# lesterphillip/SVCC23_FastSVC

Measured on AMD Instinct MI355X. Metric: audio samples/sec (24 kHz) FastSVC generator fwd, higher is better.
Workload: dtype bf16 (bf16 MFMA products, f32 accumulate; bf16 storage); 1 GPU; cfg3: 64 x 10 s utterances per GPU, F=1500 frames, T=240000 samples, generator fastsvc.yaml (144->[192,96,48,24], x[2,4,4,5]), spk_emb on; global_batch=64, utterance_samples=240000, parallelism=utterance-parallel x1

## Files before the change

### include/fastsvc_hip.h

```cpp
#ifndef FASTSVC_HIP_H
#define FASTSVC_HIP_H

#include <stddef.h>
#include <stdint.h>

#ifdef __cplusplus
extern "C" {
#endif

#define FASTSVC_ABI_VERSION 1
#define FASTSVC_MAX_STAGES 8

enum {
    FASTSVC_OK = 0,
    FASTSVC_E_INVALID = -1,
    FASTSVC_E_MISSING = -2,
    FASTSVC_E_WORKSPACE = -3,
    FASTSVC_E_HIP = -4,
    FASTSVC_E_UNSUPPORTED = -5
};

typedef struct fastsvc_config {
    int32_t in_channels;
    int32_t n_stages;
    int32_t mid_channels[FASTSVC_MAX_STAGES];
    int32_t upsampling_scales[FASTSVC_MAX_STAGES];
    int32_t out_channels;
    int32_t spk_emb_size;
    int32_t use_spk_emb;
} fastsvc_config;

typedef struct fastsvc_tensor {
    const char* name;
    const float* data;
    int64_t numel;
} fastsvc_tensor;

typedef struct fastsvc_plan fastsvc_plan;

int fastsvc_abi_version(void);
const char* fastsvc_last_error(void);

int fastsvc_plan_create(const fastsvc_config* cfg, fastsvc_plan** out_plan);
void fastsvc_plan_destroy(fastsvc_plan* plan);

int fastsvc_plan_set_storage(fastsvc_plan* plan, int32_t dtype);
int fastsvc_plan_get_storage(const fastsvc_plan* plan);

size_t fastsvc_weight_blob_bytes(const fastsvc_plan* plan);

int fastsvc_pack_weights(const fastsvc_plan* plan, const fastsvc_tensor* tensors, int32_t n_tensors,
                         void* host_blob);

size_t fastsvc_pack_device_scratch_bytes(const fastsvc_plan* plan);
int fastsvc_pack_device_launch_count(const fastsvc_plan* plan);
int fastsvc_pack_weights_device(const fastsvc_plan* plan, const fastsvc_tensor* tensors, int32_t n_tensors,
                                void* dev_blob, void* scratch, size_t scratch_bytes, void* stream);

int fastsvc_plan_set_workspace_mode(fastsvc_plan* plan, int32_t compact);

size_t fastsvc_workspace_bytes(const fastsvc_plan* plan, int32_t B, int32_t F);

int fastsvc_forward(const fastsvc_plan* plan, const void* dev_blob,
                    const float* ppg, const float* sine, const float* lft, const float* spk_emb,
                    float* out, int32_t B, int32_t F, const int32_t* lengths,
                    void* workspace, size_t workspace_bytes, void* stream);

int fastsvc_stream_prepare(void* stream);

int fastsvc_stream_release(void* stream);
// ... 122 lines not shown
```

### svcc23_fastsvc_amd/csrc/fastsvc_hx.hip

```cpp
#include "fastsvc_kernels.h"

namespace fastsvc {
#ifdef FASTSVC_ACT_2B
namespace FASTSVC_ACT_NS {
#endif

#include "fastsvc_device.inc"

#include "fastsvc_hx_common.inc"

template <int MW, int NW, bool RELOAD, bool OPT_LAST = false, int NS = 3 * MW * HX_NP, int SOFF = 0, bool ADV = true, bool HOLD = false>
__device__ __forceinline__ void hx_unit_direct(f32x4 (&acc)[NW][MW], const unsigned char* tile, const int (&aoff)[3],
                                               int lo_off, HxWeightStream<NS>& ws, bool do_last = true, bool hold = false) {
    constexpr int NSTEP = 3 * NW;
    constexpr int PF = HX_NP == 1 ? (MW >= 3 ? 2 : 3) : 1;
    HxFrag a[PF + 1];
    #pragma unroll
    for (int q = 0; q < PF && q < NSTEP; ++q) a[q] = hx_read(tile, aoff[q / NW] + (q % NW) * 16 * HX_ROW, lo_off);
    #pragma unroll
    for (int s = 0; s < NSTEP; ++s) {
        const int tap = s / NW, n = s % NW;
        if (s + PF < NSTEP) {
            a[(s + PF) % (PF + 1)] = hx_read(tile, aoff[(s + PF) / NW] + ((s + PF) % NW) * 16 * HX_ROW, lo_off);
            __builtin_amdgcn_sched_barrier(0);
// ... 436 lines not shown
            v += __builtin_bit_cast(float, __builtin_amdgcn_mov_dpp(__builtin_bit_cast(int, v), 0x4E, 0xF, 0xF, true));
            v += __builtin_bit_cast(float, __builtin_amdgcn_mov_dpp(__builtin_bit_cast(int, v), 0x141, 0xF, 0xF, true));
            v += __builtin_bit_cast(float, __builtin_amdgcn_mov_dpp(__builtin_bit_cast(int, v), 0x140, 0xF, 0xF, true));
            s[e] = v;
        }
        const int t = PAIRS ? tcol0 + (n >> 1) * 32 + (lane >> 4) * 8 + (n & 1) * 4 : tcol0 + n * 16 + (lane >> 4) * 4;
        buf_store4(yr, ((lane & 15) == 0 && t < p.T) ? t * 4 : OOB_OFF, s + bias);
    }
}

#ifndef FASTSVC_HX_W8
#define FASTSVC_HX_W8 1
#endif
constexpr bool hx_w8(int MODE, bool tailk, int S) {
    return FASTSVC_HX_W8 != 0 && HX_NP == 1 && !tailk && (MODE == MODE_DIRECT || MODE == MODE_POLY || (MODE == MODE_DEC2 && S == 2));
}
#ifndef FASTSVC_HX_CARRY
#define FASTSVC_HX_CARRY 1
#endif
constexpr bool hx_carry(int MODE, bool tailk, int S, int NT) {
    return FASTSVC_HX_CARRY != 0 && hx_w8(MODE, tailk, S) && MODE == MODE_DIRECT && S == 1 && NT == 128;
}

template <int MW, int NW, int WM, int WN, int MODE, int EPI, int S, bool WSTATIC, bool TAILK = false>
__global__ __launch_bounds__(512, (hx_min_waves<MW, NW, MODE, EPI, S, TAILK>()))
void conv_hx_kernel(const ConvParams p0) {
    constexpr bool UPH = MODE == MODE_UPHEAD;
    constexpr bool POLY = MODE == MODE_POLY, DEC2 = MODE == MODE_DEC2, CHAIN = MODE == MODE_CHAIN || MODE == MODE_CHAIN1 || UPH;
    constexpr bool IN1 = MODE == MODE_CHAIN1;
    constexpr bool WLB = MODE == MODE_CHAIN && S == 2;
    constexpr bool XR = MODE == MODE_DIRECT && S > 1;
    constexpr int NT = 16 * NW * WN;
    constexpr int NTV = CHAIN ? NT + 16 : NT;
    constexpr int HB = CHAIN ? 4 : 0;
    constexpr int NPROD_T = 256;
    constexpr bool W8 = hx_w8(MODE, TAILK, S);
    constexpr int SPARE = W8 ? 8 : 4;
    constexpr int MAXW = NTV + (MODE == MODE_DIRECT ? (W8 ? 64 : 56) : (W8 ? 16 : 8));
    constexpr int ITEMS = (MAXW + NPROD_T - 1) / NPROD_T;
    constexpr int NWS = DEC2 ? 4 : 3;
    constexpr int NVAR = DEC2 ? 2 : 1;
    constexpr int NSLOT = NWS * MW * HX_NP;
    constexpr bool TRACKS = AMAX_TRACK && ((CHAIN && MODE != MODE_UPHEAD) || (MODE == MODE_DIRECT && (EPI == EPI_RES || EPI == EPI_RANK1)));
    extern __shared__ __attribute__((aligned(16))) unsigned char smem_raw[];

    const int tid = threadIdx.x;
// ... 5 lines not shown
    const int wave_n = cw - wave_m * WN;
    const int z = blockIdx.z;
    const int sig = z / p0.B;
    const int b = z - sig * p0.B;
    ConvParams p = p0;
    if (p0.lens) {
        const int frames = p0.lens[b];
        p.T = frames * p0.len_mul;
        p.x_T = frames * p0.xlen_mul;
    }
    const int mg = blockIdx.y * WM + wave_m;
    const bool active = !producer && mg < p.ngroups;
    const int halo = (MODE == MODE_DIRECT || CHAIN) ? p.dil : 1;
    const int halo_al = W8 ? ((halo + 7) & ~7) : ((halo + 3) & ~3);
    const int W = NTV + 2 * halo_al;
    const int nch = p.nch32;
    const int CINp = nch * HX_KC;
    const int flags = p.flags;
    const int ntx = (p.T + NT - 1) / NT;
    const int tile0 = blockIdx.x * p.tpw;
    const int ntiles = min(p.tpw, ntx - tile0);
    if (ntiles <= 0) return;
    const int nunits = ntiles * (XR ? 2 * nch : nch);
#ifdef FASTSVC_TIMELINE
    const int wg_lin = blockIdx.x + gridDim.x * (blockIdx.y + gridDim.y * blockIdx.z);
    unsigned long long* tlw = (p.tl && wg_lin < p.tl_wgs) ? p.tl + ((long)wg_lin * 8 + wave) * 64 : nullptr;
    int tli = 0;
    auto stamp = [&](int tag) {
        if (tlw && lane == 0 && tli < 62) { tlw[tli++] = ((unsigned long long)tag << 56) | (__builtin_readcyclecounter() & 0x00ffffffffffffffull); }
    };
    stamp(1);
    if (tlw && lane == 0) {
        tlw[62] = __builtin_amdgcn_s_getreg(4 | (0 << 6) | (31 << 11));
        tlw[63] = __builtin_amdgcn_s_getreg(20 | (0 << 6) | (31 << 11));
    }
#else
    auto stamp = [](int) {};
#endif

    if constexpr (hx_min_waves<MW, NW, MODE, EPI, S, TAILK>() >= 4) {
        const int wg_id = blockIdx.x + gridDim.x * (blockIdx.y + gridDim.y * blockIdx.z);
        if ((wg_id >> 8) & 1) {
            for (int k = 0; k < p.stagger; ++k) __builtin_amdgcn_s_sleep(16);
        }
    }
    double* sstat = reinterpret_cast<double*>(smem_raw);
// ... 465 lines not shown
                    #pragma unroll
                    for (int m = 0; m < MW; ++m) { s1p[m] = 0.f; s2p[m] = 0.f; }
                    if (pact) P2.request(p, Rp, mg, tcolw, lane);
                    __syncthreads();
                    if (pact) {
                        P2.run(p, Rp, Pw, s1p, s2p, mg, tcolw, lane);
                        if (flags & F_STATS) {
                            #pragma unroll
                            for (int m = hx_poly_mc<MW>(); m < MW; ++m) {
                                if (lane < 16) {
                                    const int slot = ((wave_m * MW + m) * 16 + lane) * 2;
                                    atomicAdd(&sstat[slot + 0], (double)s1p[m]);
                                    atomicAdd(&sstat[slot + 1], (double)s2p[m]);
                                }
                            }
                        }
                    }
                }
            }
#endif
        };
        pwin_t pa[ITEMS][8], pb[ITEMS][8];
        unsigned oka = 0, okb = 0;
        bool carried = false;
#ifdef FASTSVC_ACT_2B
        if constexpr (hx_carry(MODE, TAILK, S, NT)) {
            carried = p.tpw > 1 && nch <= 2 && 2 * halo_al <= NT && 8 * halo_al <= NPROD_T;
            if (carried) {
                const int f_pair = ptid & 15, f_oct = ptid >> 4;
                const int f_row = 2 * halo_al + 8 * f_oct;
                auto ploadF = [&](int un, act4_t (&px)[4], unsigned& nv) {
                    const int tl = l_tl, ch = l_ch;
                    pos_next(l_tl, l_ch);
                    const int t = (tile0 + tl) * NT - halo_al + f_row;
                    const int soff = ch * HX_KC * p.ldx * 4;
                    const int rows_left = p.CIN - ch * HX_KC;
                    const bool live = ((unsigned)t < (unsigned)p.T) & (un < nunits) & !(FASTSVC_DBG_ON(p, DBG_NO_LOAD));
                    nv = live ? (unsigned)min(8, p.T - t) : 0u;
                    #pragma unroll
                    for (int c = 0; c < 2; ++c) {
                        const int r = f_pair * 2 + c;
                        typedef unsigned u32x4w __attribute__((ext_vector_type(4)));
                        const u32x4w w = __builtin_amdgcn_raw_buffer_load_b128(xr, (live & (r < rows_left)) ? (r * p.ldx + t) * 2 : OOB_OFF, soff >> 1, FASTSVC_LD_AUX);
                        px[2 * c] = act4_t{w.x, w.y};
                        px[2 * c + 1] = act4_t{w.z, w.w};
                    }
                };
                auto pcommitF = [&](const act4_t (&pw)[4], unsigned nvi, unsigned char* tile) {
                    if (FASTSVC_DBG_ON(p, DBG_NO_COMMIT)) return;
                    const int ch = c_ch;
// ... 11 lines not shown
                    }
                    #pragma unroll
                    for (int j = 0; j < 8; ++j) {
                        float e[2];
                        #pragma unroll
                        for (int c = 0; c < 2; ++c) e[c] = px[2 * c + (j >> 2)][j & 3] * A[c] + Bc[c];
                        if (j >= 4 && row_end) {
                            #pragma unroll
                            for (int c = 0; c < 2; ++c) e[c] = nvi > 4 ? e[c] : 0.f;
                        }
                        #pragma unroll
                        for (int c = 0; c < 2; ++c) e[c] = fmaxf(e[c], e[c] * slope);
                        *reinterpret_cast<unsigned*>(tile + hx_lds_off(f_row + j, f_pair >> 2) + (f_pair & 3) * 4) = a16_pack2(e[0], e[1]);
                        __builtin_amdgcn_sched_barrier(0);
                    }
                };
                const bool c_live = ptid < 8 * halo_al;
                const int c_src = NT * HX_ROW + (c_live ? ptid : 0) * 16;
                const int c_dst = c_live ? ptid * 16 : W * HX_ROW + (ptid & 31) * 16;
                auto cread = [&](const unsigned char* buf) -> u32x4 { return *reinterpret_cast<const u32x4*>(buf + c_src); };
                auto cwrite = [&](unsigned char* buf, const u32x4& v) { *reinterpret_cast<u32x4*>(buf + c_dst) = v; };
                act4_t fa[4], fb[4];
                unsigned na = 0, nb = 0;
                if (nch == 1) {
                    pload(0, pa, oka);
                    ploadF(1, fb, nb);
                    stamp(2);
                    setup_shared();
                    pcommit(0, pa, oka, tiles);
                    stamp(3);
                    __syncthreads();
                    stamp(4);
                    for (int u = 0; u < nunits; u += 2) {
                        const u32x4 ca = cread(tiles);
                        ploadF(u + 2, fa, na);
                        stamp(9);
                        cwrite(tiles + bufsz, ca);
                        pcommitF(fb, nb, tiles + bufsz);
                        stamp(5);
                        __syncthreads();
                        stamp(6);
                        const u32x4 cb = cread(tiles + bufsz);
                        ploadF(u + 3, fb, nb);
                        stamp(9);
                        cwrite(tiles, cb);
                        pcommitF(fa, na, tiles);
                        stamp(5);
// ... 26 lines not shown
                    stamp(6);
                    for (int u = 2; u < nunits; u += 2) {
                        ca = cread(tiles);
                        ploadF(u + 2, fa, na);
                        stamp(9);
                        cwrite(tiles + bufsz, cb);
                        pcommitF(fb, nb, tiles + bufsz);
                        stamp(5);
                        __syncthreads();
                        stamp(6);
                        cb = cread(tiles + bufsz);
                        ploadF(u + 3, fb, nb);
                        stamp(9);
                        cwrite(tiles, ca);
                        pcommitF(fa, na, tiles);
                        stamp(5);
                        __syncthreads();
                        stamp(6);
                    }
                }
            }
        }
#endif
        if (!carried) {
        pload(0, pa, oka);
        pload(1, pb, okb);
        stamp(2);
        setup_shared();
        if constexpr (IN1 && HX_NP == 2) {
            #pragma unroll
            for (int c = 0; c < 8; ++c) { i1w[c][0] *= sx; i1w[c][1] *= sx; i1w[c][2] *= sx; i1b[c] *= sx; }
        }
        pcommit(0, pa, oka, tiles);
        stamp(3);
        __syncthreads();
        stamp(4);
        for (int u = 0; u < nunits; u += 2) {
            pload(u + 2, pa, oka);
            stamp(9);
            pcommit(u + 1, pb, okb, tiles + bufsz);
            stamp(5);
            ppass2(u);
            __syncthreads();
            if (CHAIN && (u % nch) == nch - 1) __syncthreads();
            stamp(6);
            pload(u + 3, pb, okb);
            stamp(9);
// ... 447 lines not shown
                }
                stamp(8);
                __syncthreads();
                stamp(6);
            }
        }
        if constexpr (TRACKS) amax_flush(p, R, &s_amax, &s_cnt, 4, sig, b, lane, blockIdx.x);
        if constexpr (GSTAT || TWO) {
            if ((flags & F_STATS) && !(FASTSVC_DBG_ON(p, DBG_NO_EPILOGUE))) {
                #pragma unroll
                for (int m = 0; m < MW; ++m) {
                    double a1 = g1[GSTAT ? m : 0], a2 = g2[GSTAT ? m : 0];
                    if constexpr (TWO) { a1 = Gw[(2 * m) * 64]; a2 = Gw[(2 * m + 1) * 64]; }
                    a1 += __shfl_xor(a1, 16); a2 += __shfl_xor(a2, 16);
                    a1 += __shfl_xor(a1, 32); a2 += __shfl_xor(a2, 32);
                    if (active && lane < 16) {
                        const int slot = ((wave_m * MW + m) * 16 + lane) * 2;
                        atomicAdd(&sstat[slot + 0], a1);
                        atomicAdd(&sstat[slot + 1], a2);
                    }
                }
            }
        }
        if (nunits & 1) __syncthreads();
    }
    if ((flags & F_STATS) && !(FASTSVC_DBG_ON(p, DBG_NO_EPILOGUE))) {
        __syncthreads();
        for (int i = tid; i < 2 * 16 * MW * WM; i += 512) {
            const int co = blockIdx.y * (WM * MW * 16) + (i >> 1);
            if (co < p.COUT) atomicAdd(&p.st_out[((long)b * p.COUT + co) * 2 + (i & 1)], sstat[i]);
        }
    }
}

constexpr size_t HX_STATIC_LDS = 4096;
template <auto KERNEL>
static hipError_t hx_launch_instance(dim3 grid, size_t smem, hipStream_t stream, const ConvParams& p) {
    if (smem + HX_STATIC_LDS > 64 * 1024) {
        static const hipError_t attr = hipFuncSetAttribute(reinterpret_cast<const void*>(KERNEL),
                                                           hipFuncAttributeMaxDynamicSharedMemorySize, 160 * 1024 - HX_STATIC_LDS);
        if (attr != hipSuccess) return attr;
    }
    hipLaunchKernelGGL(KERNEL, grid, dim3(512), smem, stream, p);
    return hipGetLastError();
}

// ... 171 lines not shown
```

### svcc23_fastsvc_amd/csrc/fastsvc_kernels.h

```cpp
#pragma once
#include <hip/hip_runtime.h>
#include <stdint.h>

#if defined(FASTSVC_ACT_BF16) && defined(FASTSVC_ACT_F16)
#error "FASTSVC_ACT_BF16 and FASTSVC_ACT_F16 exclude each other"
#endif
#if defined(FASTSVC_ACT_BF16)
#define FASTSVC_ACT_2B 1
#define FASTSVC_ACT_NS bf16
#elif defined(FASTSVC_ACT_F16)
#define FASTSVC_ACT_2B 1
#define FASTSVC_ACT_NS f16
#endif

namespace fastsvc {

enum : int {
    MODE_DIRECT = 0,
    MODE_DECIMATE = 1,
    MODE_STRETCH = 2,
    MODE_POLY = 3,
    MODE_WINO = 4,
    MODE_DEC2 = 5,
    MODE_CHAIN = 6,
// ... 62 lines not shown
    long bias2_sig;
    const float* res;
    long res_sig, res_b;
    const float* r1x;
    long r1x_sig, r1x_b;
    const float* r1w;
    const float* r1b;
    long r1_sig;
    const float* ss_in;
    long ss_in_b;
    const double* st_in;
    const float* spk;
    const float* ss_out;
    long ss_out_b;
    double* st_out;
    int ntaps, dil, mode, s, flags;
    int B;
    int xs;
    int ps;
    int ldx, ldy;
    const int* lens;
    int len_mul, xlen_mul;
    int frames_ld;
    unsigned long long* tl;
    int tl_wgs;
    int vec;
    int tpw;
    int dbg;
};

struct CondStage0Params {
    const float* x;
    long x_sig, x_b;
    int B, C, T, ld;
    const int* lens;
    int len_mul;
    const float* in1_w[2];
    const float* in1_b[2];
    const float* r1w[2];
    const float* r1b[2];
    const void* w[3][2];
    const float* bias[3][2];
    const float* winv[3][2];
    const float* bnd[4][2];
    const float* bnd_r[2];
    const float* cbnd[2];
// ... 125 lines not shown
```

### svcc23_fastsvc_amd/csrc/fastsvc_plan.cpp

```cpp
#include <hip/hip_runtime.h>

#include <algorithm>
#include <chrono>
#include <cmath>
#include <cstddef>
#include <cstdio>
#include <cstdlib>
#include <cstring>
#include <functional>
#include <map>
#include <mutex>
#include <thread>
#include <type_traits>
#include <atomic>
#include <string>
#include <unordered_map>
#include <vector>

#include "fastsvc_hip.h"
#include "fastsvc_kernels.h"
#include "fastsvc_pack.h"

using namespace fastsvc;

// ... 3 lines not shown

int fail(int code, const std::string& msg) {
    g_err = msg;
    return code;
}

inline size_t align_up(size_t v, size_t a) { return (v + a - 1) / a * a; }

struct Switches {
    static int num(const char* name, int dflt) { const char* v = std::getenv(name); return v ? std::atoi(v) : dflt; }
    static double real(const char* name, double dflt) { const char* v = std::getenv(name); return v ? std::atof(v) : dflt; }
    static bool given(const char* name) { return std::getenv(name) != nullptr; }
    const int hx = num("FASTSVC_HX", 1);
    const int wx = num("FASTSVC_WX", 1);
    const int wino = num("FASTSVC_WINO", -1);
    const int chain = num("FASTSVC_CHAIN", 1);
    const int uphead = num("FASTSVC_UPHEAD", 1);
    const int d3x = num("FASTSVC_D3X", 1);
    const bool no_poly = given("FASTSVC_NO_POLY");
    const bool no_dec2 = given("FASTSVC_NO_DEC2");
    const bool no_fuse_last = given("FASTSVC_NO_FUSE_LAST");
    const int prior = num("FASTSVC_PRIOR", 1);
    const double startup_us = real("FASTSVC_STARTUP_US", 4.0);
    const int stagger = num("FASTSVC_STAGGER", 2);
    const int dbg = num("FASTSVC_DBG", 0);
    const int cond = num("FASTSVC_COND", 1);
    const int cond_pipe = num("FASTSVC_COND_PIPE", 1);
    const int cond_small = num("FASTSVC_COND_SMALL", -1);
    const int cond_tpw = num("FASTSVC_COND_TPW", 0);
    const int cond1_tpw = num("FASTSVC_COND1_TPW", 0);
    const int cond_dbg = num("FASTSVC_COND_DBG", 0);
    const bool cond_trace = given("FASTSVC_COND_TRACE");
    const bool no_amax_scan = given("FASTSVC_NO_AMAX_SCAN");
    const bool serial = given("FASTSVC_SERIAL");
    const int streams = num("FASTSVC_STREAMS", -1);
    const double fork_join_limit_us = real("FASTSVC_FORK_JOIN_LIMIT_US", 40.0);
    const bool stream_debug = given("FASTSVC_STREAM_DEBUG");
    const int pack_threads = num("FASTSVC_PACK_THREADS", 0);
    const bool pack_debug = given("FASTSVC_PACK_DEBUG");
    const bool verbose_shapes = given("FASTSVC_VERBOSE_SHAPES");
};
const Switches& env() {
    static const Switches s;
    return s;
}

// ... 127 lines not shown
}

struct fastsvc_plan {
    fastsvc_config cfg;
    int n = 0;
    std::vector<int> down_scales;
    std::vector<DownStage> down;
    std::vector<UpStage> up;
    RawParam last;
    size_t blob_floats = 0;
    std::vector<std::pair<PackedConv*, PackSource>> pack_jobs;
    struct ChainJob { PackedConv* c; std::string first, second, in1; };
    std::vector<ChainJob> chain_jobs;
    struct FilmChainJob { PackedConv* c; std::string conv[2]; PackSource heads; int C; };
    std::vector<FilmChainJob> film_chain_jobs;
    struct UpHeadJob { PackedConv* c; std::string first, res, up; int cin, C; };
    std::vector<UpHeadJob> up_head_jobs;
    struct XrJob { PackedConv* c; std::string conv, res; };
    std::vector<XrJob> xr_jobs;
    std::vector<RawParam*> raw_jobs;
    std::vector<int> cond_bound_jobs;
    double flops_per_sample = 0.0;
    int storage = 0;
    bool compact = false;
    struct Choice { int NW, WM, WN, tpw, algo; };
    mutable std::mutex tune_mu;
    mutable std::map<std::string, Choice> tuned;
    mutable std::map<std::string, Choice> priors;
    mutable std::vector<double> pack_cost;
    PackTable pk;
    mutable std::once_flag pk_once;
    mutable void* pk_pinned = nullptr;
    ~fastsvc_plan() { if (pk_pinned) (void)hipHostFree(pk_pinned); }

    bool prior_for(const char* layer, int B, int T, bool two_byte, Choice& out) const {
        const size_t ln = std::strlen(layer);
        double best = 1e30;
        bool found = false;
        for (const auto& kv : tuned) {
            const std::string& k = kv.first;
            if (k.size() <= ln + 1 || k.compare(0, ln, layer) != 0 || k[ln] != '|') continue;
            int b = 0, t = 0;
            char tail = 0;
            const int n = std::sscanf(k.c_str() + ln + 1, "%d|%d|%c", &b, &t, &tail);
            if (n < 2 || b <= 0 || t <= 0 || (n == 3) != two_byte) continue;
            const double d = std::fabs(std::log((double)b * t / ((double)B * T))) + 0.25 * std::fabs(std::log((double)t / T));
// ... 1389 lines not shown
    if (hipGetDevice(&dev) != hipSuccess) return 0;
    ExecCtx* c = nullptr;
    {
        std::lock_guard<std::mutex> lock(g_ctx_mu);
        auto it = g_ctxs.find(std::make_pair(dev, stream));
        if (it == g_ctxs.end()) return 0;
        c = it->second;
        g_ctxs.erase(it);
    }
    {
        std::lock_guard<std::mutex> busy(c->busy);
        for (hipStream_t a : c->aux)
            if (a) { (void)hipStreamSynchronize(a); (void)hipStreamDestroy(a); }
        for (hipEvent_t e : c->ev)
            if (e) (void)hipEventDestroy(e);
    }
    delete c;
    return 1;
}

struct CallCtx {
    const fastsvc_plan* plan = nullptr;
    int storage = 0;
    bool tuning = false;
    int trials = 0;
    bool exact_f32 = false;
};

#ifdef FASTSVC_TIMELINE
template <class LaunchFn>
bool timeline_launch(const char* layer, ConvParams& p, long wgs, int nchunks, const ConvLaunch& L, hipStream_t stream,
                     LaunchFn&& fn, hipError_t& err) {
    const char* want = std::getenv("FASTSVC_TIMELINE_LAYER");
    const char* out = std::getenv("FASTSVC_TIMELINE_OUT");
    if (!want || !out || std::strcmp(want, layer) != 0) return false;
    const long cap = wgs < 8192 ? wgs : 8192;
    unsigned long long* dbuf = nullptr;
    const size_t bytes = (size_t)cap * 8 * 64 * sizeof(unsigned long long);
    if (hipMalloc(&dbuf, bytes) != hipSuccess) { err = hipErrorOutOfMemory; return true; }
    hipMemsetAsync(dbuf, 0, bytes, stream);
    p.tl = dbuf; p.tl_wgs = (int)cap;
    err = fn();
    if (err != hipSuccess) return true;
    hipStreamSynchronize(stream);
    std::vector<unsigned long long> host((size_t)cap * 8 * 64);
    hipMemcpy(host.data(), dbuf, bytes, hipMemcpyDeviceToHost);
// ... 893 lines not shown
static int forward_impl(CallCtx& cc, const fastsvc_plan* plan, const void* dev_blob,
                    const float* ppg, const float* sine, const float* lft, const float* spk_emb,
                    float* out, int32_t B, int32_t F, const int32_t* lengths,
                    void* workspace, size_t workspace_bytes, void* stream_, Profiler* prof) {
    if (!plan || !dev_blob || !ppg || !sine || !lft || !out || !workspace)
        return fail(FASTSVC_E_INVALID, "null argument");
    if (B < 1 || F < 1) return fail(FASTSVC_E_INVALID, "B and F must be >= 1");
    const fastsvc_plan& P = *plan;
    if (P.storage != 0) {
        const std::string mode = P.storage == 2 ? "float16 storage" : "bfloat16 storage";
        if (F % 4 != 0) return fail(FASTSVC_E_UNSUPPORTED, mode + " needs a frame count that is a multiple of 4");
        for (int k = 0; k < P.n; ++k)
            if (P.down[k].c2[0].KC != 24 || P.up[k].d3.KC != 24 || P.up[k].first.KC != 24)
                return fail(FASTSVC_E_UNSUPPORTED, mode + " needs the pipelined kernels (24-channel K chunks)");
        if (P.n > 1 && !P.down[1].rc1[0].dec2) return fail(FASTSVC_E_UNSUPPORTED, mode + " needs the fused decimating pair");
    }
    if (spk_emb && !P.cfg.use_spk_emb)
        return fail(FASTSVC_E_INVALID, "spk_emb given but the generator was built with use_spk_emb=False");
    const Workspace ws = layout_workspace(P, B, F);
    if (workspace_bytes < ws.bytes) return fail(FASTSVC_E_WORKSPACE, "workspace too small");
    hipStream_t stream = static_cast<hipStream_t>(stream_);
    cc.plan = plan;
    cc.storage = plan->storage;
    cc.exact_f32 = plan->storage == 0 && F <= 4;
    int64_t hop_all = 1;
    for (int i = 0; i < plan->n; ++i) hop_all *= plan->cfg.upsampling_scales[i];
    int streams_mask = env().serial ? 0 : env().streams >= 0 ? (env().streams & 3) : ((int64_t)B * F * hop_all >= 150000 ? 2 : 0);
    ExecCtx* ctx = (streams_mask == 0 || cc.tuning || prof) ? nullptr : exec_ctx_for(stream);
    std::unique_lock<std::mutex> ctx_lock;
    if (ctx) {
        ctx_lock = std::unique_lock<std::mutex>(ctx->busy);
        ensure_measured(stream, ctx);
        if (env().streams < 0 && !ctx->pays) { ctx_lock.unlock(); ctx_lock = std::unique_lock<std::mutex>(); ctx = nullptr; streams_mask = 0; }
    }
    hipStream_t s_film = (ctx && (streams_mask & 2)) ? ctx->aux[0] : stream;
    hipStream_t s_side = (ctx && (streams_mask & 1)) ? ctx->aux[1] : stream;
    int evi = 0;
    auto order_after = [&](hipStream_t from, hipStream_t to) -> hipError_t {
        if (from == to || !ctx) return hipSuccess;
        hipEvent_t e = ctx->ev[evi++ % ctx->ev.size()];
        hipError_t r = hipEventRecord(e, from);
        if (r != hipSuccess) return r;
        return hipStreamWaitEvent(to, e, 0);
    };
    std::vector<hipEvent_t> ss_ready(P.n, nullptr);
    const float* blob = static_cast<const float*>(dev_blob);
// ... 57 lines not shown
                                      4.0 * (spk_c * P.cfg.spk_emb_size + (double)B * P.cfg.spk_emb_size + spk_c * B)));
        HIP_TRY(launch_spk_proj(spk_emb, blocks, n, B, P.cfg.spk_emb_size, s_pre));
        if (prof) HIP_TRY(prof->end());
    }

    long Tk = T;
    const float* hprev = sigbuf;
    int Cprev = 1;
    long Tprev = T;
    bool hprev_compact = false;
    for (int k = 0; k < n; ++k) {
        const DownStage& d = P.down[k];
        Tk = Tk / d.scale;
        const std::string s = std::to_string(k);
        float* c1 = buf("down_c1." + s);
        float* c2 = buf("down_c2." + s);
        float* h = buf("down_h." + s);
        const long tsig = (long)B * d.C * Tk;
        const long tb = (long)d.C * Tk;
        ConvParams base;
        std::memset(&base, 0, sizeof(base));
        base.B = B; base.T = (int)Tk; base.s = 1; base.mode = MODE_DIRECT;
        base.lens = lengths; base.frames_ld = F;
        base.amax_in_sig = B; base.amax_out_sig = B;
        float* am_prev = k == 0 ? amax_inb : am("down_h." + std::to_string(k - 1));
        float* am_h = am("down_h." + s);
        const float* bnd_c1 = blob + (k == 0 ? d.c1_raw[0].bnd_off : d.c1[0].bnd_off);
        const long bnd_c1_sig = k == 0 ? (long)(d.c1_raw[1].bnd_off - d.c1_raw[0].bnd_off) : d.c1[0].bnd_pair;
        auto stage_unfused = [&](Profiler* pr) -> int {
            if (k == 0) {
                if (pr) HIP_TRY(pr->begin(stream, "down.0.c1", "in1_conv", 2.0 * 3 * d.C * (double)Tk * B * 2,
                                              4.0 * (1.0 + d.C) * (double)Tk * B * 2));
                HIP_TRY(FASTSVC_BY_STORAGE(P.storage, launch_in1_conv)(sigbuf, sig_stride, blob + d.c1_raw[0].w_off, blob + d.c1_raw[0].b_off,
                                        (long)(d.c1_raw[1].w_off - d.c1_raw[0].w_off),
                                        (long)(d.c1_raw[1].b_off - d.c1_raw[0].b_off), c1, 2, B, d.C, (int)Tk,
                                        lengths, (int)(Tk / F), stream, nullptr));
                if (pr) HIP_TRY(pr->end());
            } else {
                float* r = buf("down_r." + s);
                ConvParams p = base;
                p.x = hprev; p.x_sig = (long)B * Cprev * Tprev; p.x_b = (long)Cprev * Tprev; p.x_T = (int)Tprev;
                p.mode = MODE_DECIMATE; p.s = hprev_compact ? 1 : d.scale;
                p.amax_in = am_prev;
                if (d.rc1[0].dec2 && !env().no_dec2) {
                    p.mode = MODE_DEC2;
                    p.y = c1; p.y_sig = tsig; p.y_b = tb;
// ... 149 lines not shown
        if (env().no_fuse_last || (table_entry(P, key, ch) && ch.algo != 3)) last_fusable = false;
    }
    for (int i = 0; i < n; ++i) {
        const UpStage& u = P.up[i];
        const int k = n - 1 - i;
        const long Tout = Tin * u.scale;
        const std::string s = std::to_string(i);
        float* a = buf("up." + s + ".a");
        float* xr = buf("up." + s + ".xr");
        float* u1 = buf("up." + s + ".u1");
        float* xm = buf("up." + s + ".xmid");
        float* u2 = buf("up." + s + ".u2");
        float* u3 = buf("up." + s + ".u3");
        float* xo = buf("up." + s + ".out");
        float* pb = buf("up." + s + ".spk");
        double* st = reinterpret_cast<double*>(buf("up." + s + ".stats"));
        const float* ss = buf("ss." + std::to_string(k));
        const long cb = (long)u.C * Tout;
        const long stn = (long)B * u.C * 2;
        ConvParams base;
        std::memset(&base, 0, sizeof(base));
        base.B = B; base.s = 1; base.mode = MODE_DIRECT;
        base.lens = lengths; base.frames_ld = F;
        const int aff_out = F_AFF_OUT | (spk ? F_STATS : 0);
        const int pre = F_PRE_LRELU | (spk ? F_PRE_NORM : 0);

        if (ss_ready[k]) HIP_TRY(hipStreamWaitEvent(stream, ss_ready[k], 0));

        float* am_x = i == 0 ? amax_inb + 2 * B * 256 : am("up." + std::to_string(i - 1) + ".out");
        float* am_p = am("up." + s + ".spk");
        bool head_fused = false;
        {
            ConvParams ph = base;
            ph.x = x; ph.x_b = (long)Cx * Tin; ph.x_T = (int)Tin;
            ph.y = xr; ph.y_b = cb; ph.y2 = u1; ph.y2_b = cb;
            ph.flags = F_POST_LRELU | aff_out;
            ph.ss_out = ss; ph.ss_out_b = 2 * cb; ph.st_out = st;
            ph.amax_in = am_x;
            HIP_TRY(run_uphead(cc, u, blob, ph, stream, prof, ("up." + s + ".head").c_str(), head_fused));
        }
        ConvParams pd3 = base;
        pd3.x = u1; pd3.x_b = cb; pd3.x_T = (int)Tout; pd3.T = (int)Tout;
        pd3.flags = pre | aff_out; pd3.st_in = st; pd3.spk = pb;
        pd3.amax_in = spk ? am_p : nullptr;
        pd3.no_hx = (!spk && P.storage == 0) ? 1 : 0;
        pd3.y = xm; pd3.y_b = cb; pd3.y2 = u2; pd3.y2_b = cb;
// ... 108 lines not shown
        if (f16_lo) f16_lo[i] = f32_to_f16(x[i] - f16_to_f32(hi));
        if (bf16) bf16[i] = f32_to_bf16(x[i]);
    }
}

int fastsvc_stream_prepare(void* stream) {
    ExecCtx* c = exec_ctx_for(static_cast<hipStream_t>(stream));
    if (!c) return fail(FASTSVC_E_HIP, "could not create the helper streams / events");
    std::lock_guard<std::mutex> busy(c->busy);
    ensure_measured(static_cast<hipStream_t>(stream), c);
    return FASTSVC_OK;
}

int fastsvc_stream_release(void* stream) { return exec_ctx_release(static_cast<hipStream_t>(stream)); }

int fastsvc_plan_set_storage(fastsvc_plan* plan, int32_t dtype) {
    if (!plan || (dtype != 0 && dtype != 1 && dtype != 2)) return fail(FASTSVC_E_INVALID, "storage dtype must be 0 (float32), 1 (bfloat16) or 2 (float16)");
    plan->storage = dtype;
    return FASTSVC_OK;
}

int fastsvc_plan_get_storage(const fastsvc_plan* plan) { return plan ? plan->storage : 0; }

int fastsvc_tuned_count(const fastsvc_plan* plan) {
    if (!plan) return 0;
    std::lock_guard<std::mutex> lock(plan->tune_mu);
    return (int)plan->tuned.size();
}

int fastsvc_tuned_get(const fastsvc_plan* plan, int32_t index, char* key_out, int32_t shape_out[5]) {
    if (!plan || !key_out || !shape_out) return fail(FASTSVC_E_INVALID, "null argument");
    std::lock_guard<std::mutex> lock(plan->tune_mu);
    if (index < 0 || index >= (int32_t)plan->tuned.size()) return fail(FASTSVC_E_INVALID, "index out of range");
    auto it = plan->tuned.begin();
    std::advance(it, index);
    std::snprintf(key_out, 96, "%s", it->first.c_str());
    shape_out[0] = it->second.NW; shape_out[1] = it->second.WM; shape_out[2] = it->second.WN; shape_out[3] = it->second.tpw;
    shape_out[4] = it->second.algo;
    return FASTSVC_OK;
}

int fastsvc_tuned_set(const fastsvc_plan* plan, const char* key, const int32_t shape[5]) {
    if (!plan || !key || !shape) return fail(FASTSVC_E_INVALID, "null argument");
    if (std::strlen(key) >= 96) return fail(FASTSVC_E_INVALID, "key too long");
    table_record(*plan, key, fastsvc_plan::Choice{shape[0], shape[1], shape[2], shape[3], shape[4]});
    return FASTSVC_OK;
// ... 46 lines not shown
```

### svcc23_fastsvc_amd/engine.py

```python
from __future__ import annotations

import ctypes
import json
import os
from typing import Dict, Mapping, Optional, Sequence, Tuple

import numpy as np
import torch

from .synth import GeneratorConfig

_LIB = None
_LIB_PATH = os.environ.get("FASTSVC_HIP_LIB") or \
    os.path.join(os.path.dirname(os.path.abspath(__file__)), "libfastsvc_hip.so")
MAX_STAGES = 8
STORAGE_CODES = {"float32": 0, "bfloat16": 1, "float16": 2}
STORAGE_DTYPES = {"float32": torch.float32, "bfloat16": torch.bfloat16, "float16": torch.float16}
TUNED_TABLE_PATH = os.path.join(os.path.dirname(os.path.abspath(__file__)), "tuned_mi355x.json")

ABI_SYMBOLS = (
    "fastsvc_abi_version", "fastsvc_last_error", "fastsvc_plan_create", "fastsvc_plan_destroy",
    "fastsvc_plan_set_storage", "fastsvc_plan_get_storage",
    "fastsvc_weight_blob_bytes", "fastsvc_pack_weights", "fastsvc_workspace_bytes",
    "fastsvc_pack_device_scratch_bytes", "fastsvc_pack_device_launch_count", "fastsvc_pack_weights_device",
    "fastsvc_forward", "fastsvc_autotune", "fastsvc_tuned_count", "fastsvc_tuned_get", "fastsvc_tuned_set",
    "fastsvc_forward_profile", "fastsvc_workspace_tap", "fastsvc_forward_launch_count",
    "fastsvc_flops_per_sample", "fastsvc_signal_scratch_bytes", "fastsvc_signal_generate",
    "fastsvc_stream_prepare", "fastsvc_stream_release", "fastsvc_split_half", "fastsvc_plan_set_workspace_mode",
    "fastsvc_loudness_frames", "fastsvc_loudness_scratch_bytes", "fastsvc_loudness_extract",
    "fastsvc_gather_padded", "fastsvc_gather_time_major", "fastsvc_pcm16_pack",
    "fastsvc_pcm16_pack_checked", "fastsvc_output_check",
    "fastsvc_collate_launch_count", "fastsvc_collate_crops",
    "fastsvc_fanout_launch_count", "fastsvc_fanout_assemble",
    "fastsvc_stft_loss_scratch_bytes", "fastsvc_stft_loss_forward", "fastsvc_stft_loss_backward",
    "fastsvc_conv1d_forward", "fastsvc_conv1d_backward_weight", "fastsvc_conv1d_backward_weight_scratch_bytes",
    "fastsvc_film_norm_forward", "fastsvc_film_norm_backward", "fastsvc_weight_norm_forward", "fastsvc_weight_norm_backward",
    "fastsvc_gconv1d_supported", "fastsvc_gconv1d_forward", "fastsvc_gconv1d_backward_data",
    "fastsvc_gconv1d_backward_weight_scratch_bytes", "fastsvc_gconv1d_backward_weight",
)


class FastSVCError(RuntimeError):
    pass


# ... 22 lines not shown
    return _LIB_PATH


def load_library():
    global _LIB
    if _LIB is not None:
        return _LIB
    if not os.path.exists(_LIB_PATH):
        raise FastSVCError(
            f"{_LIB_PATH} not found: build it with `python -m svcc23_fastsvc_amd.build` "
            "(hipcc --offload-arch=gfx950). There is no CPU fallback for this path.")
    lib = ctypes.CDLL(_LIB_PATH)
    vp, sz, i32, i64 = ctypes.c_void_p, ctypes.c_size_t, ctypes.c_int32, ctypes.c_int64
    lib.fastsvc_abi_version.restype = ctypes.c_int
    lib.fastsvc_last_error.restype = ctypes.c_char_p
    lib.fastsvc_plan_create.argtypes = [ctypes.POINTER(_Config), ctypes.POINTER(vp)]
    lib.fastsvc_plan_create.restype = ctypes.c_int
    lib.fastsvc_plan_destroy.argtypes = [vp]
    lib.fastsvc_plan_destroy.restype = None
    lib.fastsvc_plan_set_storage.argtypes = [vp, i32]
    lib.fastsvc_plan_set_storage.restype = ctypes.c_int
    lib.fastsvc_plan_get_storage.argtypes = [vp]
    lib.fastsvc_plan_get_storage.restype = ctypes.c_int
    lib.fastsvc_weight_blob_bytes.argtypes = [vp]
    lib.fastsvc_weight_blob_bytes.restype = sz
    lib.fastsvc_pack_weights.argtypes = [vp, ctypes.POINTER(_Tensor), i32, vp]
    lib.fastsvc_pack_weights.restype = ctypes.c_int
    lib.fastsvc_pack_device_scratch_bytes.argtypes = [vp]
    lib.fastsvc_pack_device_scratch_bytes.restype = sz
    lib.fastsvc_pack_device_launch_count.argtypes = [vp]
    lib.fastsvc_pack_device_launch_count.restype = ctypes.c_int
    lib.fastsvc_pack_weights_device.argtypes = [vp, ctypes.POINTER(_Tensor), i32, vp, vp, sz, vp]
    lib.fastsvc_pack_weights_device.restype = ctypes.c_int
    lib.fastsvc_workspace_bytes.argtypes = [vp, i32, i32]
    lib.fastsvc_workspace_bytes.restype = sz
    lib.fastsvc_forward.argtypes = [vp, vp, vp, vp, vp, vp, vp, i32, i32, vp, vp, sz, vp]
    lib.fastsvc_forward.restype = ctypes.c_int
    lib.fastsvc_loudness_frames.argtypes = [i32, i32]
    lib.fastsvc_loudness_frames.restype = i32
    lib.fastsvc_loudness_scratch_bytes.argtypes = [i32, i32, i32]
    lib.fastsvc_loudness_scratch_bytes.restype = sz
    lib.fastsvc_loudness_extract.argtypes = [vp, vp, vp, i32, i32, i32, ctypes.c_float, vp]
    lib.fastsvc_loudness_extract.restype = ctypes.c_int
    lib.fastsvc_stft_loss_scratch_bytes.argtypes = [i32, i32, i32, vp, vp]
    lib.fastsvc_stft_loss_scratch_bytes.restype = sz
    lib.fastsvc_stft_loss_forward.argtypes = [vp, vp, i32, i32, i32, vp, vp, vp, vp, vp, vp, vp]
# ... 318 lines not shown
    us = (ctypes.c_int32 * R)(*[int(v) for v in utt])
    ss = (ctypes.c_int32 * R)(*[int(v) for v in spk])
    ptr = lambda t: ctypes.c_void_p(t.data_ptr()) if t is not None else None
    with torch.cuda.device(ppg.device):
        stream = torch.cuda.current_stream(ppg.device).cuda_stream
        _check(lib, lib.fastsvc_fanout_assemble(ptr(ppg), ppg.numel(), ptr(lft), lft.numel(), ptr(f0), f0.numel(), U,
                                                po, lo, fo, nfr, ptr(src_stats), ptr(spk_stats), ptr(spk_emb), n_spk, us, ss,
                                                *[ptr(t) for t in outs], R, C, E, hop, width, ctypes.c_void_p(stream)),
               "fastsvc_fanout_assemble")
    return tuple(outs)


def _check(lib, rc: int, what: str):
    if rc != 0:
        msg = lib.fastsvc_last_error().decode("utf-8", "replace")
        if rc == -1:
            raise ValueError(f"{what}: {msg}")
        raise FastSVCError(f"{what} failed ({rc}): {msg}")


class Plan:

    def __init__(self, cfg: GeneratorConfig, load_shipped_table: bool = True, storage: str = "float32",
                 compact_workspace: bool = False):
        if storage not in STORAGE_CODES:
            raise ValueError("storage must be 'float32', 'bfloat16' or 'float16'")
        self.storage = storage
        self.cfg = cfg
        self.lib = load_library()
        if cfg.n_stages > MAX_STAGES or len(cfg.upsampling_scales) != cfg.n_stages:
            raise ValueError("mid_channels / upsampling_scales must have equal length <= 8")
        c = _Config()
        c.in_channels = cfg.in_channels
        c.n_stages = cfg.n_stages
        for i in range(cfg.n_stages):
            c.mid_channels[i] = cfg.mid_channels[i]
            c.upsampling_scales[i] = cfg.upsampling_scales[i]
        c.out_channels = cfg.out_channels
        c.spk_emb_size = cfg.spk_emb_size
        c.use_spk_emb = 1 if cfg.use_spk_emb else 0
        handle = ctypes.c_void_p()
        _check(self.lib, self.lib.fastsvc_plan_create(ctypes.byref(c), ctypes.byref(handle)), "fastsvc_plan_create")
        self._h = handle
        if storage != "float32":
            _check(self.lib, self.lib.fastsvc_plan_set_storage(handle, STORAGE_CODES[storage]), "fastsvc_plan_set_storage")
        self.compact_workspace = bool(compact_workspace)
        if compact_workspace:
            _check(self.lib, self.lib.fastsvc_plan_set_workspace_mode(handle, 1), "fastsvc_plan_set_workspace_mode")
        self.last_autotune_trials = 0
        self.pad_odd_lengths = True
        if load_shipped_table:
            self.load_tuned_file(TUNED_TABLE_PATH, missing_ok=True)

    def config_signature(self) -> str:
        c = self.cfg
        return "in%d_mid%s_up%s_out%d_spk%d" % (c.in_channels, "-".join(map(str, c.mid_channels)),
                                                "-".join(map(str, c.upsampling_scales)), c.out_channels,
                                                c.spk_emb_size if c.use_spk_emb else 0)

    def tuned_shapes(self) -> dict:
        out = {}
        key = ctypes.create_string_buffer(96)
        shape = (ctypes.c_int32 * 5)()
        for i in range(int(self.lib.fastsvc_tuned_count(self._h))):
            _check(self.lib, self.lib.fastsvc_tuned_get(self._h, i, key, ctypes.byref(shape)), "fastsvc_tuned_get")
            out[key.value.decode()] = [int(v) for v in shape]
        return out

# ... 353 lines not shown
```

Measured before the change: 1.832 billion samples/s.

## Deepen producer-wave global prefetch pipeline in hx conv kernel to PF stages

Adds a deeper software pipeline (3 or 4 in-flight global loads) for the producer waves that stage activation windows into LDS in the hx conv kernel, covering both the carried-halo path and the plain path. It is enabled by default for the one-operand W8 instances, except direct strided and large affine-epilogue instances. A plan/env knob can force the old depth-2 scheme. The aim is to hide more global-memory latency per unit. The cost is more producer registers, larger unrolled code, and extra barrier bookkeeping for the tail.

```diff
diff --git a/include/fastsvc_hip.h b/include/fastsvc_hip.h
--- a/include/fastsvc_hip.h
+++ b/include/fastsvc_hip.h
@@ -46,6 +46,9 @@
 
 int fastsvc_plan_set_storage(fastsvc_plan* plan, int32_t dtype);
 int fastsvc_plan_get_storage(const fastsvc_plan* plan);
+
+int fastsvc_plan_set_hx_prefetch(fastsvc_plan* plan, int32_t depth);
+int fastsvc_plan_get_hx_prefetch(const fastsvc_plan* plan);
 
 size_t fastsvc_weight_blob_bytes(const fastsvc_plan* plan);
 
diff --git a/svcc23_fastsvc_amd/csrc/fastsvc_hx.hip b/svcc23_fastsvc_amd/csrc/fastsvc_hx.hip
--- a/svcc23_fastsvc_amd/csrc/fastsvc_hx.hip
+++ b/svcc23_fastsvc_amd/csrc/fastsvc_hx.hip
@@ -482,6 +482,15 @@
     return FASTSVC_HX_CARRY != 0 && hx_w8(MODE, tailk, S) && MODE == MODE_DIRECT && S == 1 && NT == 128;
 }
 
+#ifndef FASTSVC_HX_PF
+#define FASTSVC_HX_PF 4
+#endif
+constexpr int hx_pf(int MW, int NW, int MODE, int EPI, bool tailk, int S) {
+    if (FASTSVC_HX_PF <= 2 || !hx_w8(MODE, tailk, S) || (MODE == MODE_DIRECT && S > 1)) return 2;
+    if (MODE == MODE_DIRECT && EPI == EPI_AFF && MW * NW >= 18) return 2;
+    return FASTSVC_HX_PF == 3 ? 3 : 4;
+}
+
 template <int MW, int NW, int WM, int WN, int MODE, int EPI, int S, bool WSTATIC, bool TAILK = false>
 __global__ __launch_bounds__(512, (hx_min_waves<MW, NW, MODE, EPI, S, TAILK>()))
 void conv_hx_kernel(const ConvParams p0) {
@@ -533,6 +542,11 @@
     const int ntiles = min(p.tpw, ntx - tile0);
     if (ntiles <= 0) return;
     const int nunits = ntiles * (XR ? 2 * nch : nch);
+    constexpr int PF = hx_pf(MW, NW, MODE, EPI, TAILK, S);
+    constexpr int PFU = (PF & 1) ? 2 * PF : PF;
+    static_assert(PF == 2 || !(CHAIN || XR || TAILK), "the deep staging loops exist for the one-operand window instances only");
+    const bool deep = PF > 2 && p.pf != 2;
+    const bool carried = hx_carry(MODE, TAILK, S, NT) && p.tpw > 1 && nch <= 2 && 2 * halo_al <= NT && 8 * halo_al <= NPROD_T;
 #ifdef FASTSVC_TIMELINE
     const int wg_lin = blockIdx.x + gridDim.x * (blockIdx.y + gridDim.y * blockIdx.z);
     unsigned long long* tlw = (p.tl && wg_lin < p.tl_wgs) ? p.tl + ((long)wg_lin * 8 + wave) * 64 : nullptr;
@@ -1044,10 +1058,8 @@
         };
         pwin_t pa[ITEMS][8], pb[ITEMS][8];
         unsigned oka = 0, okb = 0;
-        bool carried = false;
 #ifdef FASTSVC_ACT_2B
         if constexpr (hx_carry(MODE, TAILK, S, NT)) {
-            carried = p.tpw > 1 && nch <= 2 && 2 * halo_al <= NT && 8 * halo_al <= NPROD_T;
             if (carried) {
                 const int f_pair = ptid & 15, f_oct = ptid >> 4;
                 const int f_row = 2 * halo_al + 8 * f_oct;
@@ -1105,7 +1117,78 @@
                 auto cwrite = [&](unsigned char* buf, const u32x4& v) { *reinterpret_cast<u32x4*>(buf + c_dst) = v; };
                 act4_t fa[4], fb[4];
                 unsigned na = 0, nb = 0;
-                if (nch == 1) {
+                if constexpr (PF > 2) {
+                if (deep) {
+                    act4_t f[PF][4];
+                    unsigned nf[PF];
+                    if (nch == 1) {
+                        pload(0, pa, oka);
+                        #pragma unroll
+                        for (int k = 1; k < PF; ++k) ploadF(k, f[k], nf[k]);
+                        stamp(2);
+                        setup_shared();
+                        pcommit(0, pa, oka, tiles);
+                        stamp(3);
+                        __syncthreads();
+                        stamp(4);
+                        for (int u = 0; u < nunits; u += PFU) {
+                            #pragma unroll
+                            for (int k = 0; k < PFU; ++k) {
+                                const u32x4 cv = cread(tiles + (k & 1) * bufsz);
+                                ploadF(u + k + PF, f[k % PF], nf[k % PF]);
+                                stamp(9);
+                                cwrite(tiles + ((k + 1) & 1) * bufsz, cv);
+                                pcommitF(f[(k + 1) % PF], nf[(k + 1) % PF], tiles + ((k + 1) & 1) * bufsz);
+                                stamp(5);
+                                __syncthreads();
+                                stamp(6);
+                            }
+                        }
+                    } else {
+                        u32x4 cc[2];
+                        pload(0, pa, oka);
+                        pload(1, pb, okb);
+                        #pragma unroll
+                        for (int k = 2; k < PF; ++k) ploadF(k, f[k], nf[k]);
+                        stamp(2);
+                        setup_shared();
+                        pcommit(0, pa, oka, tiles);
+                        stamp(3);
+                        __syncthreads();
+                        stamp(4);
+                        cc[0] = cread(tiles);
+                        ploadF(PF, f[0], nf[0]);
+                        stamp(9);
+                        pcommit(1, pb, okb, tiles + bufsz);
+                        stamp(5);
+                        __syncthreads();
+                        stamp(6);
+                        cc[1] = cread(tiles + bufsz);
+                        ploadF(PF + 1, f[1], nf[1]);
+                        stamp(9);
+                        cwrite(tiles, cc[0]);
+                        pcommitF(f[2 % PF], nf[2 % PF], tiles);
+                        stamp(5);
+                        __syncthreads();
+                        stamp(6);
+                        for (int u = 2; u < nunits; u += PFU) {
+                            #pragma unroll
+                            for (int k = 0; k < PFU; ++k) {
+                                cc[k & 1] = cread(tiles + (k & 1) * bufsz);
+                                ploadF(u + k + PF, f[(2 + k) % PF], nf[(2 + k) % PF]);
+                                stamp(9);
+                                cwrite(tiles + ((k + 1) & 1) * bufsz, cc[(k + 1) & 1]);
+                                pcommitF(f[(3 + k) % PF], nf[(3 + k) % PF], tiles + ((k + 1) & 1) * bufsz);
+                                stamp(5);
+                                __syncthreads();
+                                stamp(6);
+                            }
+                        }
+                    }
+                }
+                }
+                if (deep) {
+                } else if (nch == 1) {
                     pload(0, pa, oka);
                     ploadF(1, fb, nb);
                     stamp(2);
@@ -1178,7 +1261,33 @@
             }
         }
 #endif
-        if (!carried) {
+        if constexpr (PF > 2) {
+        if (!carried && deep) {
+            pwin_t ps[PF][ITEMS][8];
+            unsigned ok[PF];
+            #pragma unroll
+            for (int k = 0; k < PF; ++k) pload(k, ps[k], ok[k]);
+            stamp(2);
+            setup_shared();
+            pcommit(0, ps[0], ok[0], tiles);
+            stamp(3);
+            __syncthreads();
+            stamp(4);
+            for (int u = 0; u < nunits; u += PFU) {
+                #pragma unroll
+                for (int k = 0; k < PFU; ++k) {
+                    pload(u + k + PF, ps[k % PF], ok[k % PF]);
+                    stamp(9);
+                    pcommit(u + k + 1, ps[(k + 1) % PF], ok[(k + 1) % PF], tiles + ((k + 1) & 1) * bufsz);
+                    stamp(5);
+                    ppass2(u + k);
+                    __syncthreads();
+                    stamp(6);
+                }
+            }
+        }
+        }
+        if (!carried && !deep) {
         pload(0, pa, oka);
         pload(1, pb, okb);
         stamp(2);
@@ -1672,6 +1781,10 @@
                 }
             }
         }
+        if (deep) {
+            const int peel = (carried && nch == 2) ? 2 : 0;
+            for (int k = (nunits - peel) % PFU; k != 0 && k < PFU; ++k) __syncthreads();
+        } else
         if (nunits & 1) __syncthreads();
     }
     if ((flags & F_STATS) && !(FASTSVC_DBG_ON(p, DBG_NO_EPILOGUE))) {
diff --git a/svcc23_fastsvc_amd/csrc/fastsvc_kernels.h b/svcc23_fastsvc_amd/csrc/fastsvc_kernels.h
--- a/svcc23_fastsvc_amd/csrc/fastsvc_kernels.h
+++ b/svcc23_fastsvc_amd/csrc/fastsvc_kernels.h
@@ -108,6 +108,7 @@
     const int* lens;
     int len_mul, xlen_mul;
     int frames_ld;
+    int pf;
     unsigned long long* tl;
     int tl_wgs;
     int vec;
diff --git a/svcc23_fastsvc_amd/csrc/fastsvc_plan.cpp b/svcc23_fastsvc_amd/csrc/fastsvc_plan.cpp
--- a/svcc23_fastsvc_amd/csrc/fastsvc_plan.cpp
+++ b/svcc23_fastsvc_amd/csrc/fastsvc_plan.cpp
@@ -49,6 +49,7 @@
     const bool no_fuse_last = given("FASTSVC_NO_FUSE_LAST");
     const int prior = num("FASTSVC_PRIOR", 1);
     const double startup_us = real("FASTSVC_STARTUP_US", 4.0);
+    const int hx_pf = num("FASTSVC_HX_PF", 0);
     const int stagger = num("FASTSVC_STAGGER", 2);
     const int dbg = num("FASTSVC_DBG", 0);
     const int cond = num("FASTSVC_COND", 1);
@@ -222,6 +223,7 @@
     std::vector<int> cond_bound_jobs;
     double flops_per_sample = 0.0;
     int storage = 0;
+    int hx_prefetch = 0;
     bool compact = false;
     struct Choice { int NW, WM, WN, tpw, algo; };
     mutable std::mutex tune_mu;
@@ -1657,6 +1659,7 @@
 struct CallCtx {
     const fastsvc_plan* plan = nullptr;
     int storage = 0;
+    int hx_pf = 0;
     bool tuning = false;
     int trials = 0;
     bool exact_f32 = false;
@@ -2596,6 +2599,7 @@
     hipStream_t stream = static_cast<hipStream_t>(stream_);
     cc.plan = plan;
     cc.storage = plan->storage;
+    cc.hx_pf = env().hx_pf == 2 ? 2 : plan->hx_prefetch;
     cc.exact_f32 = plan->storage == 0 && F <= 4;
     int64_t hop_all = 1;
     for (int i = 0; i < plan->n; ++i) hop_all *= plan->cfg.upsampling_scales[i];
@@ -2699,6 +2703,7 @@
         std::memset(&base, 0, sizeof(base));
         base.B = B; base.T = (int)Tk; base.s = 1; base.mode = MODE_DIRECT;
         base.lens = lengths; base.frames_ld = F;
+        base.pf = cc.hx_pf;
         base.amax_in_sig = B; base.amax_out_sig = B;
         float* am_prev = k == 0 ? amax_inb : am("down_h." + std::to_string(k - 1));
         float* am_h = am("down_h." + s);
@@ -2894,6 +2899,7 @@
         std::memset(&base, 0, sizeof(base));
         base.B = B; base.s = 1; base.mode = MODE_DIRECT;
         base.lens = lengths; base.frames_ld = F;
+        base.pf = cc.hx_pf;
         const int aff_out = F_AFF_OUT | (spk ? F_STATS : 0);
         const int pre = F_PRE_LRELU | (spk ? F_PRE_NORM : 0);
 
@@ -3048,6 +3054,14 @@
 
 int fastsvc_plan_get_storage(const fastsvc_plan* plan) { return plan ? plan->storage : 0; }
 
+int fastsvc_plan_set_hx_prefetch(fastsvc_plan* plan, int32_t depth) {
+    if (!plan || (depth != 0 && depth != 2)) return fail(FASTSVC_E_INVALID, "hx prefetch depth must be 0 (each kernel instance's own) or 2");
+    plan->hx_prefetch = depth;
+    return FASTSVC_OK;
+}
+
+int fastsvc_plan_get_hx_prefetch(const fastsvc_plan* plan) { return plan ? plan->hx_prefetch : 0; }
+
 int fastsvc_tuned_count(const fastsvc_plan* plan) {
     if (!plan) return 0;
     std::lock_guard<std::mutex> lock(plan->tune_mu);
diff --git a/svcc23_fastsvc_amd/engine.py b/svcc23_fastsvc_amd/engine.py
--- a/svcc23_fastsvc_amd/engine.py
+++ b/svcc23_fastsvc_amd/engine.py
@@ -20,7 +20,7 @@
 
 ABI_SYMBOLS = (
     "fastsvc_abi_version", "fastsvc_last_error", "fastsvc_plan_create", "fastsvc_plan_destroy",
-    "fastsvc_plan_set_storage", "fastsvc_plan_get_storage",
+    "fastsvc_plan_set_storage", "fastsvc_plan_get_storage", "fastsvc_plan_set_hx_prefetch", "fastsvc_plan_get_hx_prefetch",
     "fastsvc_weight_blob_bytes", "fastsvc_pack_weights", "fastsvc_workspace_bytes",
     "fastsvc_pack_device_scratch_bytes", "fastsvc_pack_device_launch_count", "fastsvc_pack_weights_device",
     "fastsvc_forward", "fastsvc_autotune", "fastsvc_tuned_count", "fastsvc_tuned_get", "fastsvc_tuned_set",
@@ -89,6 +89,10 @@
     lib.fastsvc_plan_set_storage.restype = ctypes.c_int
     lib.fastsvc_plan_get_storage.argtypes = [vp]
     lib.fastsvc_plan_get_storage.restype = ctypes.c_int
+    lib.fastsvc_plan_set_hx_prefetch.argtypes = [vp, i32]
+    lib.fastsvc_plan_set_hx_prefetch.restype = ctypes.c_int
+    lib.fastsvc_plan_get_hx_prefetch.argtypes = [vp]
+    lib.fastsvc_plan_get_hx_prefetch.restype = ctypes.c_int
     lib.fastsvc_weight_blob_bytes.argtypes = [vp]
     lib.fastsvc_weight_blob_bytes.restype = sz
     lib.fastsvc_pack_weights.argtypes = [vp, ctypes.POINTER(_Tensor), i32, vp]
@@ -453,7 +457,7 @@
 class Plan:
 
     def __init__(self, cfg: GeneratorConfig, load_shipped_table: bool = True, storage: str = "float32",
-                 compact_workspace: bool = False):
+                 compact_workspace: bool = False, hx_prefetch: int = 0):
         if storage not in STORAGE_CODES:
             raise ValueError("storage must be 'float32', 'bfloat16' or 'float16'")
         self.storage = storage
@@ -475,6 +479,9 @@
         self._h = handle
         if storage != "float32":
             _check(self.lib, self.lib.fastsvc_plan_set_storage(handle, STORAGE_CODES[storage]), "fastsvc_plan_set_storage")
+        self.hx_prefetch = int(hx_prefetch)
+        if hx_prefetch:
+            _check(self.lib, self.lib.fastsvc_plan_set_hx_prefetch(handle, int(hx_prefetch)), "fastsvc_plan_set_hx_prefetch")
         self.compact_workspace = bool(compact_workspace)
         if compact_workspace:
             _check(self.lib, self.lib.fastsvc_plan_set_workspace_mode(handle, 1), "fastsvc_plan_set_workspace_mode")
```

Result: no change. 1.828 billion samples/s (-0.2%).
